# lab-cosmo/torch-pme

Hardware: AMD Instinct MI355X
Metric: atom-steps/sec (energy+forces) (higher is better)
Workload: dtype f32

## Files before the change

torch-pme_amd/csrc/bricks_device.h:

```cpp
#ifndef MIPME_BRICKS_DEVICE_H
#define MIPME_BRICKS_DEVICE_H
#include <algorithm>
#include <cmath>
#include <cstdlib>

#include <rocprim/device/device_radix_sort.hpp>

#include "host.h"
#include <map>
#include <utility>

#include "rows_body.h"
#include "fft_lds.h"

namespace mipme {

static constexpr int BRICK = 8;
static constexpr int BRICK_PTS = BRICK * BRICK * BRICK;

#define MIPME_SGPR_CAP __attribute__((amdgpu_num_sgpr(80)))
static inline int spread_stage_rows(int order, size_t real_bytes);
static inline size_t spread_row_reals(int, size_t) { return 3 * BRICK; }

struct BrickGeom {
  int nbx, nby, nbz, nb;
  int xcd;
};

static inline BrickGeom make_brick_geom(const mipme_mesh_t* m) {
  BrickGeom b;
  b.nbx = (m->nx + BRICK - 1) / BRICK;
  b.nby = (m->ny + BRICK - 1) / BRICK;
  b.nbz = (m->nz + BRICK - 1) / BRICK;
  b.nb = b.nbx * b.nby * b.nbz;
  b.xcd = 1;
  return b;
}
static inline unsigned brick_grid(const BrickGeom& b) { return b.xcd ? pad8(unsigned(b.nb)) : unsigned(b.nb); }
__device__ __forceinline__ unsigned brick_of(const BrickGeom& b, unsigned wg) {
  return b.xcd ? xcd_contiguous(wg, unsigned(b.nb)) : wg;
}

__device__ __forceinline__ int wrap1(int a, int n) {
  a += a < 0 ? n : 0;
  return a >= n ? a - n : a;
}

struct BinsLayout {
  size_t snap, over_brick, rec, wts, codes, qs, plist, pover, wmax, epart, dst, det, det_sort_bytes, total;
  int cap;
  int pcap;
  int64_t slots;
};

static bool deterministic_mode() {
  static const bool on = env_flag("MIPME_DETERMINISTIC", false);
  return on;
}
static constexpr int kRowsPerSpreadBlock = 512 / kRowLanes;
static constexpr int kSpreadWaves = 512 / 64;

static inline int bin_capacity(int nb, int64_t N) {
  const int64_t mean = (N + nb - 1) / nb;
  int64_t cap = (4 * mean + 8 + 7) / 8 * 8;
  const int64_t all = (N + 7) / 8 * 8;
  if (cap > all) cap = all;
  return int(cap < 8 ? 8 : cap);
}

template <int N, typename T>
constexpr int wts_stride() {
  constexpr int V = 16 / int(sizeof(T));
  return (6 * N + V - 1) / V * V;
}
static inline size_t wts_stride_rt(int order, size_t elem) { return (6 * size_t(order) * elem + 15) / 16 * 16 / elem; }

template <int N, typename T>
__device__ __forceinline__ void store_slot_weights(T* __restrict__ wr, const T (&wx)[N], const T (&wy)[N], const T (&wz)[N],
                                                   const T (&dwx)[N], const T (&dwy)[N], const T (&dwz)[N]) {
  constexpr int W = wts_stride<N, T>(), V = 16 / int(sizeof(T));
  struct alignas(16) Chunk {
    T e[V];
  };
  T v[W];
#pragma unroll
  for (int t = 0; t < N; ++t) {
    v[t] = wx[t];
    v[N + t] = wy[t];
    v[2 * N + t] = wz[t];
    v[3 * N + t] = dwx[t];
    v[4 * N + t] = dwy[t];
    v[5 * N + t] = dwz[t];
  }
#pragma unroll
  for (int t = 6 * N; t < W; ++t) v[t] = T(0);
  Chunk* d = reinterpret_cast<Chunk*>(wr);
#pragma unroll
  for (int k = 0; k < W / V; ++k) {
    Chunk c;
#pragma unroll
    for (int e = 0; e < V; ++e) c.e[e] = v[k * V + e];
    d[k] = c;
  }
}

template <int N, typename T>
constexpr int plane_entry_words() {
  constexpr int V = 16 / int(sizeof(T));
  return (3 + N + V - 1) / V * V;
}
static inline size_t plane_entry_bytes_rt(int order, size_t elem) { return ((3 + size_t(order)) * elem + 15) / 16 * 16; }
static constexpr int kPlanePackBits = 10;

static int plane_list_capacity(const mipme_mesh_t* m, int64_t N, int dtype);
static inline BinsLayout bins_layout(const mipme_mesh_t* m, int64_t N, int dtype) {
  const BrickGeom b = make_brick_geom(m);
  const size_t s = dtype == MIPME_F32 ? 4 : 8;
  auto al = [](size_t x) { return (x + 255) & ~size_t(255); };
  BinsLayout l;
  l.cap = bin_capacity(b.nb, N);
  l.slots = int64_t(b.nb) * l.cap + N;
  size_t off = 0;
  l.snap = off;       off += al(sizeof(int) * size_t(b.nb + 1));
  l.over_brick = off; off += al(sizeof(int) * size_t(N));
  l.rec = off;        off += al(sizeof(int4) * size_t(l.slots));
  l.wts = off;        off += al(wts_stride_rt(m->order, s) * s * size_t(l.slots));
  l.codes = off;      off += al(size_t(l.slots));
  l.qs = off;         off += al(s * size_t(l.slots));
  l.pcap = plane_list_capacity(m, N, dtype);
  l.plist = off;      off += al(plane_entry_bytes_rt(m->order, s) * size_t(l.pcap) * size_t(l.pcap ? m->nx * kPlaneSub : 0));
  l.pover = off;      off += al(plane_entry_bytes_rt(m->order, s) * size_t(l.pcap ? N : 0));
  l.wmax = off;       off += al(sizeof(float) * size_t(l.pcap ? (N + 63) / 64 : 0));
  l.epart = off; off += al(2 * sizeof(double) * kSpreadWaves * (((size_t(N) + kRowsPerSpreadBlock - 1) / kRowsPerSpreadBlock + 1) & ~size_t(1)));
  l.dst = off;        off += al(sizeof(int) * size_t(N));
  l.det = off;
  l.det_sort_bytes = 0;
  if (deterministic_mode()) {
    size_t sb = 0;
    unsigned* nul = nullptr;
    (void)rocprim::radix_sort_pairs(nullptr, sb, nul, nul, nul, nul, size_t(N > 0 ? N : 1), 0u, 32u, hipStream_t(0), false);
    l.det_sort_bytes = sb;
    off += 6 * al(sizeof(int) * size_t(N > 0 ? N : 1)) + al(sb);
  }
  l.total = off;
  return l;
}

struct BinIndex {
  int* live;
  int* snap;
  const int* over_brick;
  int nb, cap;
  int64_t over_base;
  unsigned char* codes = nullptr;
  int* plive = nullptr;
  int pband_shift = -1;
  void* plist = nullptr;
  void* pover = nullptr;
  int pcap = 0;
  float* wmax = nullptr;
  int n_wmax = 0;
};

template <int N>
__device__ __forceinline__ unsigned reach_code(const int (&m)[3], int nx, int ny, int nz) {
  constexpr int s0 = stencil_start<N>();
  const int n[3] = {nx, ny, nz};
  unsigned code = 0;
#pragma unroll
  for (int d = 0; d < 3; ++d) {
    const int i = m[d] & (BRICK - 1), size = min(BRICK, n[d] - (m[d] & ~(BRICK - 1)));
    code |= (i + s0 < 0 ? 1u : 0u) << (2 * d);
    code |= (i + s0 + N - 1 >= size ? 2u : 0u) << (2 * d);
  }
  return code;
}

__device__ __forceinline__ void split_runtime(double u, bool even, int& m, double& x) {
  if (even) {
    const double fl = floor(u);
    m = int(fl);
    x = u - (fl + 0.5);
  } else {
    const double r = rint(u);
    m = int(r);
    x = u - r;
  }
}

template <typename T>
__device__ __forceinline__ void atom_mesh_coords(const Geom& g, bool even, const T* __restrict__ pos, int64_t i,
                                                 int (&m)[3], double (&x)[3]) {
  const double rx = double(pos[3 * i + 0]), ry = double(pos[3 * i + 1]), rz = double(pos[3 * i + 2]);
  const double u[3] = {double(g.nx) * (rx * g.inv[0] + ry * g.inv[3] + rz * g.inv[6]),
                       double(g.ny) * (rx * g.inv[1] + ry * g.inv[4] + rz * g.inv[7]),
                       double(g.nz) * (rx * g.inv[2] + ry * g.inv[5] + rz * g.inv[8])};
  const int n[3] = {g.nx, g.ny, g.nz};
#pragma unroll
  for (int d = 0; d < 3; ++d) {
    int mm;
    split_runtime(u[d], even, mm, x[d]);
    m[d] = posmod(mm, n[d]);
  }
}

static constexpr int64_t kCoalescedBinAtoms = 100000;
template <int SCHEME, int N, typename T, bool COALESCE = false, bool LEAN = false>
__device__ __forceinline__ void bin_atoms_body(const Geom& g, const BrickGeom& bg, const BinIndex& bi, int64_t Natoms,
                                               const T* __restrict__ pos, int* __restrict__ over_brick,
                                               int4* __restrict__ rec, T* __restrict__ wts, const T* __restrict__ q,
                                               AtomRecord<T>* __restrict__ atom_rec, unsigned block,
                                               const int* __restrict__ slot_of = nullptr, T* __restrict__ qs = nullptr,
                                               int* __restrict__ slot_dst = nullptr) {
  static_assert(!(LEAN && COALESCE), "the lean binning pass has no weight rows to stage");
  const int64_t i = int64_t(block) * blockDim.x + threadIdx.x;
  const bool valid = i < Natoms;
  const int lane = threadIdx.x & 63;
  int b = -1;
  int m[3] = {0, 0, 0};
  double x[3] = {0.0, 0.0, 0.0};
  if (valid) {
    atom_mesh_coords<T>(g, (N % 2) == 0, pos, i, m, x);
    b = ((m[0] / BRICK) * bg.nby + m[1] / BRICK) * bg.nbz + m[2] / BRICK;
  }
  int myslot = 0, over_k = -1;
  int pl_leader = lane, pl_rank = 0, pl_count = 0, pl_slot = -1;
  const int pl_key = bi.pband_shift >= 0 ? ((m[1] >> bi.pband_shift) & (kPlaneSub - 1))
                                         : int(((int64_t(block) * blockDim.x + threadIdx.x) >> 6) & (kPlaneSub - 1));
  const int pl_list = m[0] * kPlaneSub + pl_key;
  if (slot_of) {
    if (valid) {
      myslot = slot_of[i];
      if (myslot >= bi.cap) over_k = myslot - bi.cap;
    }
  } else {
    unsigned long long remaining = __ballot(valid);
    int my_leader = lane, my_rank = 0, my_count = 0;
    while (remaining) {
      const int leader = __ffsll((long long)remaining) - 1;
      const int b0 = __shfl(b, leader, 64);
      const unsigned long long peers = __ballot(valid && b == b0);
      if (valid && b == b0) {
        my_leader = leader;
        my_rank = __popcll(peers & ((1ull << lane) - 1ull));
        my_count = __popcll(peers);
      }
      remaining &= ~peers;
    }
    if (bi.plive && bi.wmax && qs) {
      float a = valid ? fabsf(float(q[i])) : 0.f;
      a = fmaxf(a, dpp_mov<0xB1>(a));
      a = fmaxf(a, dpp_mov<0x4E>(a));
      a = fmaxf(a, dpp_mov<0x141>(a));
      a = fmaxf(a, dpp_mov<0x140>(a));
      a = fmaxf(fmaxf(read_lane(a, 0), read_lane(a, 16)), fmaxf(read_lane(a, 32), read_lane(a, 48)));
      if (lane == 0) bi.wmax[(int64_t(block) * blockDim.x + threadIdx.x) >> 6] = a;
    }
    if (bi.plive) {
      unsigned long long rem = __ballot(valid);
      while (rem) {
        const int leader = __ffsll((long long)rem) - 1;
        const int p0 = __shfl(pl_list, leader, 64);
        const unsigned long long peers = __ballot(valid && pl_list == p0);
        if (valid && pl_list == p0) {
          pl_leader = leader;
          pl_rank = __popcll(peers & ((1ull << lane) - 1ull));
          pl_count = __popcll(peers);
        }
        rem &= ~peers;
      }
    }
    int base = 0, pbase = 0;
    if (valid && my_leader == lane) base = atomicAdd(&bi.live[b], my_count);
    if (bi.plive && valid && pl_leader == lane) pbase = atomicAdd(&bi.plive[pl_list], pl_count);
    base = __shfl(base, my_leader, 64);
    myslot = base + my_rank;
    if (bi.plive) pl_slot = __shfl(pbase, pl_leader, 64) + pl_rank;
  }
  int64_t dst = 0;
  if (valid) {
    if (myslot < bi.cap) {
      dst = int64_t(b) * bi.cap + myslot;
    } else {
      const int k = over_k >= 0 ? over_k : atomicAdd(&bi.live[bi.nb], 1);
      over_brick[k] = b;
      dst = bi.over_base + k;
    }
    if (atom_rec) {
      AtomRecord<T> r;
      r.x = pos[3 * i];
      r.y = pos[3 * i + 1];
      r.z = pos[3 * i + 2];
      r.w = q[i];
      atom_rec[i] = r;
    }
    if constexpr (LEAN) {
      slot_dst[i] = int(dst);
    } else {
      rec[dst] = make_int4(m[0], m[1], m[2], int(i));
      if (qs) qs[dst] = q[i];
      if (bi.codes && dst < bi.over_base) bi.codes[dst] = (unsigned char)reach_code<N>(m, g.nx, g.ny, g.nz);
    }
  }
  constexpr int W = wts_stride<N, T>();
  auto store_plane_entry = [&](const T (&wx)[N]) __attribute__((always_inline)) {
    if (!valid || pl_slot < 0) return;
    constexpr int EW = plane_entry_words<N, T>(), V = 16 / int(sizeof(T));
    struct alignas(16) Chunk {
      T e[V];
    };
    T* e;
    if (pl_slot < bi.pcap)
      e = (T*)bi.plist + (int64_t(pl_list) * bi.pcap + pl_slot) * EW;
    else
      e = (T*)bi.pover + int64_t(atomicAdd(&bi.plive[g.nx * kPlaneSub], 1)) * EW;
    T v[EW];
    const int packed = (m[0] << (2 * kPlanePackBits)) | (m[1] << kPlanePackBits) | m[2];
    if constexpr (sizeof(T) == 4)
      v[0] = __int_as_float(packed);
    else
      v[0] = __longlong_as_double((long long)packed);
    v[1] = T(x[1]);
    v[2] = T(x[2]);
    const T qa = q[i];
#pragma unroll
    for (int t = 0; t < N; ++t) v[3 + t] = qa * wx[t];
#pragma unroll
    for (int t = 3 + N; t < EW; ++t) v[t] = T(0);
    Chunk* d = reinterpret_cast<Chunk*>(e);
#pragma unroll
    for (int k = 0; k < EW / V; ++k) {
      Chunk c;
#pragma unroll
      for (int u = 0; u < V; ++u) c.e[u] = v[k * V + u];
      d[k] = c;
    }
  };
  constexpr bool STAGED = COALESCE && sizeof(T) * 64 * W * (256 / 64) <= 48 * 1024;
  if constexpr (STAGED) {
    __shared__ T sw[256 / 64][64 * W];
    T* mine = sw[threadIdx.x >> 6] + lane * W;
#pragma unroll
    for (int d = 0; d < 3; ++d) {
      T w[N], dw[N];
      weights_1d<SCHEME, N, true, T>(T(x[d]), w, dw);
#pragma unroll
      for (int t = 0; t < N; ++t) {
        mine[d * N + t] = w[t];
        mine[(3 + d) * N + t] = dw[t];
      }
      if (d == 0 && bi.plive) store_plane_entry(w);
    }
    __builtin_amdgcn_fence(__ATOMIC_RELEASE, "wavefront");
    __builtin_amdgcn_wave_barrier();
    constexpr int PER = 64 / W;
    const unsigned long long vmask = __ballot(valid);
    const int sub = lane / W, k = lane % W;
    const T* rows = sw[threadIdx.x >> 6];
    for (int a0 = 0; a0 < 64; a0 += PER) {
      const int j = a0 + (sub < PER ? sub : 0);
      const int64_t dj = __shfl(dst, j < 64 ? j : 0, 64);
      if (sub < PER && k < 6 * N && j < 64 && ((vmask >> j) & 1ull)) wts[dj * W + k] = rows[j * W + k];
    }
  } else if constexpr (LEAN) {
    if (!valid) return;
    T wx[N], dwx[N];
    weights_1d<SCHEME, N, false, T>(T(x[0]), wx, dwx);
    if (bi.plive) store_plane_entry(wx);
  } else {
    if (!valid) return;
    T wx[N], wy[N], wz[N], dwx[N], dwy[N], dwz[N];
    weights_1d<SCHEME, N, true, T>(T(x[0]), wx, dwx);
    weights_1d<SCHEME, N, true, T>(T(x[1]), wy, dwy);
    weights_1d<SCHEME, N, true, T>(T(x[2]), wz, dwz);
    store_slot_weights<N, T>(wts + dst * W, wx, wy, wz, dwx, dwy, dwz);
    if (bi.plive) store_plane_entry(wx);
  }
}

template <int SCHEME, int N, typename T, bool COALESCE>
__global__ __launch_bounds__(256) void bin_atoms_kernel(Geom g, BrickGeom bg, BinIndex bi, int64_t Natoms,
                                                       const T* __restrict__ pos, int* __restrict__ over_brick,
                                                       int4* __restrict__ rec, T* __restrict__ wts,
                                                       const T* __restrict__ q, AtomRecord<T>* __restrict__ atom_rec,
                                                       const int* __restrict__ slot_of, T* __restrict__ qs) {
  bin_atoms_body<SCHEME, N, T, COALESCE>(g, bg, bi, Natoms, pos, over_brick, rec, wts, q, atom_rec, blockIdx.x, slot_of, qs);
}

template <int SCHEME, int N, typename T>
__global__ __launch_bounds__(256) void bin_atoms_lean_kernel(Geom g, BrickGeom bg, BinIndex bi, int64_t Natoms,
                                                            const T* __restrict__ pos, int* __restrict__ over_brick,
                                                            const T* __restrict__ q, AtomRecord<T>* __restrict__ atom_rec,
                                                            T* __restrict__ qs, int* __restrict__ slot_dst) {
  bin_atoms_body<SCHEME, N, T, false, true>(g, bg, bi, Natoms, pos, over_brick, nullptr, nullptr, q, atom_rec, blockIdx.x, nullptr,
                                            qs, slot_dst);
}

#ifndef MIPME_SLOT_RIDER_ATOMS
#define MIPME_SLOT_RIDER_ATOMS 256
#endif
static constexpr int kSlotRiderAtoms = MIPME_SLOT_RIDER_ATOMS;
template <int SCHEME, int N, typename T>
__device__ __forceinline__ void slot_rider_body(const SlotRider& r, unsigned rider) {
  if (int(threadIdx.x) >= r.per_rider) return;
  const int64_t i = int64_t(rider) * r.per_rider + threadIdx.x;
  if (i >= r.n_atoms) return;
  const T* __restrict__ pos = static_cast<const T*>(r.pos);
  const T* __restrict__ q = static_cast<const T*>(r.q);
  const int64_t dst = r.dst[i];
  int m[3];
  double x[3];
  atom_mesh_coords<T>(r.g, (N % 2) == 0, pos, i, m, x);
  r.rec[dst] = make_int4(m[0], m[1], m[2], int(i));
  static_cast<T*>(r.qs)[dst] = q[i];
  if (dst < r.over_base) r.codes[dst] = (unsigned char)reach_code<N>(m, r.g.nx, r.g.ny, r.g.nz);
  T wx[N], wy[N], wz[N], dwx[N], dwy[N], dwz[N];
  weights_1d<SCHEME, N, true, T>(T(x[0]), wx, dwx);
  weights_1d<SCHEME, N, true, T>(T(x[1]), wy, dwy);
  weights_1d<SCHEME, N, true, T>(T(x[2]), wz, dwz);
  store_slot_weights<N, T>(static_cast<T*>(r.wts) + dst * wts_stride<N, T>(), wx, wy, wz, dwx, dwy, dwz);
}

template <typename T>
__global__ __launch_bounds__(256) void det_keys_kernel(Geom g, BrickGeom bg, bool even, int64_t Natoms, const T* __restrict__ pos,
                                                      unsigned* __restrict__ keys, unsigned* __restrict__ vals) {
  const int64_t i = int64_t(blockIdx.x) * blockDim.x + threadIdx.x;
  if (i >= Natoms) return;
  int m[3];
  double x[3];
  atom_mesh_coords<T>(g, even, pos, i, m, x);
  keys[i] = unsigned(((m[0] / BRICK) * bg.nby + m[1] / BRICK) * bg.nbz + m[2] / BRICK);
  vals[i] = unsigned(i);
}

static __global__ __launch_bounds__(256) void det_slots_kernel(int64_t Natoms, int cap, const unsigned* __restrict__ keys2,
                                                       const unsigned* __restrict__ vals2, int* __restrict__ slot_of,
                                                       int* __restrict__ over_flag, int* __restrict__ live) {
  const int64_t p = int64_t(blockIdx.x) * blockDim.x + threadIdx.x;
  if (p >= Natoms) return;
  const unsigned b = keys2[p];
  int64_t lo = 0, hi = p;
  while (lo < hi) {
    const int64_t mid = (lo + hi) >> 1;
    if (keys2[mid] < b)
      lo = mid + 1;
    else
      hi = mid;
  }
  const int slot = int(p - lo);
  slot_of[vals2[p]] = slot;
  over_flag[p] = slot >= cap ? 1 : 0;
  if (slot == 0) {
    int64_t l2 = p, h2 = Natoms;
    while (l2 < h2) {
      const int64_t mid = (l2 + h2) >> 1;
      if (keys2[mid] <= b)
        l2 = mid + 1;
      else
        h2 = mid;
    }
    live[b] = int(l2 - p);
  }
}

static __global__ __launch_bounds__(1024) void det_overflow_kernel(int64_t Natoms, int cap, int nb, const unsigned* __restrict__ vals2,
                                                           const int* __restrict__ over_flag, int* __restrict__ slot_of,
                                                           int* __restrict__ live) {
  __shared__ int part[1024];
  const int t = threadIdx.x;
  const int64_t per = (Natoms + 1023) / 1024;
  const int64_t lo = min(int64_t(t) * per, Natoms), hi = min(lo + per, Natoms);
  int sum = 0;
  for (int64_t k = lo; k < hi; ++k) sum += over_flag[k];
  part[t] = sum;
  __syncthreads();
  for (int off = 1; off < 1024; off <<= 1) {
    const int v = t >= off ? part[t - off] : 0;
    __syncthreads();
    part[t] += v;
    __syncthreads();
  }
// ... 470 lines not shown
  extern __shared__ __attribute__((aligned(16))) char smem_rows[];
  if (cs.brick) {
    const unsigned b = brick_of(sa.bg, cs.slot);
    if (cs.slot < n_pad && b < n_spread) spread_brick_body<N, T>(sa, b);
  } else if (cs.slot < n_rows_pad) {
    const unsigned r = sa.bg.xcd ? xcd_contiguous(cs.slot, n_row_blocks) : cs.slot;
    if (r < n_row_blocks) cosched_row_block<T, PFAST, COMPACT, CELL>(ra, r, smem_rows);
  }
#ifdef MIPME_WG_TIMELINE
  __syncthreads();
#endif
  MIPME_WG_STAMP(1);
}

template <int N, typename T, int PFAST, bool COMPACT, bool CELL = false>
__global__ __launch_bounds__(SPREAD_THREADS, (sizeof(T) == 4 && COMPACT) ? (CELL ? MIPME_CELL_WAVES : 6) : 1) void spread_rows_kernel(
    SpreadArgs<T> sa, FusedRowsArgs<T> ra, unsigned n_spread, unsigned pattern) {
  spread_rows_body<N, T, PFAST, COMPACT, CELL>(sa, ra, n_spread, pattern);
}
template <int N, typename T, int PFAST, bool COMPACT, bool CELL = false>
__global__ __launch_bounds__(SPREAD_THREADS, (sizeof(T) == 4 && COMPACT) ? (CELL ? MIPME_CELL_WAVES : 6) : 1) MIPME_SGPR_CAP void spread_rows_capped_kernel(
    SpreadArgs<T> sa, FusedRowsArgs<T> ra, unsigned n_spread, unsigned pattern) {
  spread_rows_body<N, T, PFAST, COMPACT, CELL>(sa, ra, n_spread, pattern);
}
template <int N, typename T, bool CELL>
constexpr bool spread_rows_sgpr_capped() {
#ifdef MIPME_SGPR_CAP_OFF
  return false;
#else
  return sizeof(T) == 4 && N == 5 && !CELL;
#endif
}

template <typename T, int PFAST, bool COMPACT, bool CELL = false>
__global__ __launch_bounds__(256) void rows_only_kernel(FusedRowsArgs<T> ra, int xcd) {
  constexpr bool F64_BODY = COMPACT && std::is_same<T, double>::value && (PFAST == 1 || PFAST == 6) && kRowLanes == 16;
  __shared__ __attribute__((aligned(16))) char tab_raw[F64_BODY ? kRowsF64LdsBytes : sizeof(AtomRecord<T>) * kShiftTableSize];
  AtomRecord<T>* tab = reinterpret_cast<AtomRecord<T>*>(tab_raw);
  constexpr int BS = 256;
  const unsigned n_row_blocks = unsigned((ra.N + BS / kRowLanes - 1) / (BS / kRowLanes));
  const unsigned r = xcd ? xcd_contiguous(blockIdx.x, n_row_blocks) : blockIdx.x;
  if (r >= n_row_blocks) return;
  if constexpr (COMPACT && std::is_same<T, float>::value) {
    if (CELL || !ra.dist_out) {
      sr_rows_pk_body<PFAST, BS, CELL>(ra, r, tab);
      return;
    }
  }
#if MIPME_ROW_LANES == 16
  if constexpr (F64_BODY) {
    if (CELL || !ra.dist_out) {
      sr_rows_f64_body<BS, CELL, PFAST>(ra, r, tab_raw);
      return;
    }
  }
#endif
  if constexpr (!CELL) sr_fused_rows_body<T, kPotForce, false, PFAST, false, true, BS, 0, COMPACT>(ra, r, tab);
}

template <typename T>
static inline bool rows_cell_supported(int pfast, int shift_format, const void* dist_out) {
  if ((shift_format & kShiftFormatMask) != kShiftTable32 || dist_out || kRowLanes != 16) return false;
  return pfast == 1 || pfast == 6;
}

template <typename T>
struct PlaneArgs {
  Cplx<T>* hat = nullptr;
  int logny = 0, loglz = 0;
  int tile_off = 0, tw_off = 0;
  int misc_off = 0;
  int parts = 1;
  Cplx<T>* hat_more = nullptr;
  int64_t more_stride = 0;
  int band_rows = 0, bands = 1;
};

static constexpr size_t kPlaneLdsCosched = 39 * 1024;
static inline size_t plane_tile_bytes(int ny, int nz, size_t real_bytes) { return 2 * real_bytes * size_t(ny) * (size_t(nz / 2) + 1); }
static inline size_t plane_tw_bytes(int ny, int nz, size_t real_bytes) {
  const size_t Lz = size_t(nz / 2), Ltab = size_t(ny) > Lz ? size_t(ny) : Lz;
  return 2 * real_bytes * (Ltab / 2 + (Lz + 1));
}
template <typename T>
static inline void plane_lds_layout(int rows, int nz, PlaneArgs<T>& pa, size_t& total, bool ystage = true) {
  const size_t acc = sizeof(double) * size_t(rows) * nz, tile = plane_tile_bytes(rows, nz, sizeof(T));
  const size_t tile_off = sizeof(T) == 4 ? 0 : acc;
  const size_t tw_off = sizeof(T) == 4 ? (acc > tile ? acc : tile) : acc + tile;
  pa.tile_off = int(tile_off);
  pa.tw_off = int(tw_off);
  pa.misc_off = int(tw_off + plane_tw_bytes(ystage ? rows : 0, nz, sizeof(T)));
  total = size_t(pa.misc_off) + 640;
}
static inline int plane_band_rows(const mipme_mesh_t* m, int dtype) {
  static const bool bands_env = env_flag("MIPME_PLANE_BANDS", true);
  for (int rows = m->ny; rows >= 4 && rows * kPlaneSub >= m->ny; rows >>= 1) {
    size_t need = 0;
    if (dtype == MIPME_F32) {
      PlaneArgs<float> pa;
      plane_lds_layout<float>(rows, m->nz, pa, need, rows == m->ny);
    } else {
      PlaneArgs<double> pa;
      plane_lds_layout<double>(rows, m->nz, pa, need, rows == m->ny);
    }
    if (need <= kPlaneLdsCosched) return rows;
    if (!bands_env) break;
  }
  return 0;
}
static inline bool plane_fits_cosched(const mipme_mesh_t* m, int dtype) { return plane_band_rows(m, dtype) == m->ny; }

static inline bool sparse_bricks(int64_t n_atoms, int nb);
static int plane_list_capacity(const mipme_mesh_t* m, int64_t N, int dtype) {
  static const bool plane_env = env_flag("MIPME_PLANE_SPREAD", true);
  if (!plane_env || deterministic_mode() || m->n_channels != 1 || N <= 0) return 0;
  const bool pow2 = (m->ny & (m->ny - 1)) == 0 && (m->nz & (m->nz - 1)) == 0 && m->nz >= 4 && m->ny >= 2;
  if (!pow2 || m->nx < 2 * BRICK) return 0;
  if (m->nx > (1 << 11) || m->ny > (1 << kPlanePackBits) || m->nz > (1 << kPlanePackBits)) return 0;
  if (sparse_bricks(N, make_brick_geom(m).nb)) return 0;
  const int band_rows = plane_band_rows(m, dtype);
  if (band_rows == 0) return 0;
  if (band_rows < m->ny && m->ny / kPlaneSub < 8) return 0;
  const int64_t lists = int64_t(m->nx) * kPlaneSub, mean = (N + lists - 1) / lists, all = (N + 15) / 16 * 16;
  int64_t cap = (4 * mean + 32 + 15) / 16 * 16;
  if (cap > all) cap = all;
  return int(cap);
}

template <int N, typename T>
struct PlaneItem {
  T vx;
  int my, mz;
  T wy[N], wz[N];
};

template <int N, typename T>
struct PlaneRaw {
  T w[plane_entry_words<N, T>()];
};

template <int N, typename T>
__device__ __forceinline__ void plane_raw_load(PlaneRaw<N, T>& r, bool ok, const T* __restrict__ base, int64_t idx) {
  constexpr int EW = plane_entry_words<N, T>(), V = 16 / int(sizeof(T));
  struct alignas(16) Chunk {
    T e[V];
  };
  const Chunk* src = reinterpret_cast<const Chunk*>(base + (ok ? idx : 0) * EW);
#pragma unroll
  for (int k = 0; k < EW / V; ++k) {
    const Chunk c = src[k];
#pragma unroll
    for (int u = 0; u < V; ++u) r.w[k * V + u] = c.e[u];
  }
#pragma unroll
  for (int t = 3; t < EW; ++t) r.w[t] = ok ? r.w[t] : T(0);
}
template <typename T>
__device__ __forceinline__ int plane_raw_packed(T w0) {
  if constexpr (sizeof(T) == 4)
    return __float_as_int(w0);
  else
    return int(__double_as_longlong(w0));
}

template <int SCHEME, int N, typename T>
__device__ __forceinline__ void plane_item_make(PlaneItem<N, T>& it, const PlaneRaw<N, T>& r, int tt, T scale) {
  const int packed = plane_raw_packed(r.w[0]);
  it.my = (packed >> kPlanePackBits) & ((1 << kPlanePackBits) - 1);
  it.mz = packed & ((1 << kPlanePackBits) - 1);
  T qwx[N], unused[N];
#pragma unroll
  for (int t = 0; t < N; ++t) qwx[t] = r.w[3 + t];
  it.vx = pick<N, T>(qwx, tt) * scale;
  weights_1d<SCHEME, N, false, T>(r.w[1], it.wy, unused);
  weights_1d<SCHEME, N, false, T>(r.w[2], it.wz, unused);
}

static constexpr unsigned kFxMagicHi = 0x43380000u;
template <int N, typename T, bool BANDED>
__device__ __forceinline__ void plane_item_scatter(double* __restrict__ acc, const Geom& g, const PlaneItem<N, T>& it, double fx_scale,
                                                   int row_lo, int rows) {
  constexpr int s0 = stencil_start<N>();
  int zo[N];
#pragma unroll
  for (int k = 0; k < N; ++k) zo[k] = wrap1(it.mz + s0 + k, g.nz);
#pragma unroll
  for (int j = 0; j < N; ++j) {
    int r = wrap1(it.my + s0 + j, g.ny);
    if constexpr (BANDED) {
      r -= row_lo;
      if (unsigned(r) >= unsigned(rows)) continue;
    }
    const int row = r * g.nz;
    const T ay = it.vx * it.wy[j];
#pragma unroll
    for (int k = 0; k < N; ++k) {
      if constexpr (sizeof(T) == 4) {
        const double t = __builtin_fma(double(ay * it.wz[k]), fx_scale, 6755399441055744.0);
        const unsigned long long bits = (unsigned long long)__double_as_longlong(t) - ((unsigned long long)kFxMagicHi << 32);
        atomicAdd(reinterpret_cast<unsigned long long*>(&acc[row + zo[k]]), bits);
      } else {
        atomicAdd(&acc[row + zo[k]], double(ay * it.wz[k]));
      }
    }
  }
}

template <int SCHEME, int N, typename T, bool BANDED = false>
__device__ __forceinline__ void plane_spread_yz_body(const SpreadArgs<T>& args, const PlaneArgs<T>& pa, unsigned item,
                                                     char* smem) {
  constexpr bool banded = BANDED;
  const int n_bands = banded ? pa.bands : 1;
  const unsigned unit = item / unsigned(pa.parts);
  const int part = int(item - unit * unsigned(pa.parts));
  const unsigned plane = banded ? unit / unsigned(n_bands) : unit;
  const int band = banded ? int(unit - plane * unsigned(n_bands)) : 0;
  const Geom& g = args.g;
  const int rows = banded ? pa.band_rows : g.ny, row_lo = band * rows;
  const BinIndex& bins = args.bins;
  const T* __restrict__ plist = (const T*)bins.plist;
  const T* __restrict__ pover = (const T*)bins.pover;
  const int tid = threadIdx.x, nthr = blockDim.x;
  constexpr int s0 = stencil_start<N>();
  MIPME_WG_PHASE(0);
  double* acc = reinterpret_cast<double*>(smem);
  const int npts = rows * g.nz;
  const int x0 = int(plane);
  const int spb = kPlaneSub / n_bands;
  const int SUBS = banded ? min(spb + 2, kPlaneSub) : kPlaneSub;
  const int sub0 = banded ? band * spb - 1 : 0;
  const int NL = N * SUBS;
  auto list_of = [&](int l) __attribute__((always_inline)) {
    return posmod(x0 - s0 - l / SUBS, g.nx) * kPlaneSub + ((sub0 + (l % SUBS)) & (kPlaneSub - 1));
  };
  int my_count = 0;
  if (tid < NL) my_count = bins.plive[list_of(tid)];
  float my_wmax = 0.f;
  if (sizeof(T) == 4 && tid < bins.n_wmax) my_wmax = bins.wmax[tid];
  for (int i = tid; i < npts; i += nthr) acc[i] = 0.0;
  const YzTile<T> yt = banded ? yz_tile_setup<T, false>(rows, g.nz, smem + pa.tile_off, smem + pa.tw_off)
                              : yz_tile_setup<T, true>(g.ny, g.nz, smem + pa.tile_off, smem + pa.tw_off);
  if (args.from_live) {
    const int n_items = g.nx * n_bands * pa.parts;
    for (int b = int(item) + tid * n_items; b <= bins.nb; b += n_items * nthr) bins.snap[b] = bin_count_of(bins, b, true);
  }
  int* lst = reinterpret_cast<int*>(smem + pa.misc_off);
  static_assert(N * kPlaneSub < 64, "bookkeeping of the plane lists");
  double* fxs = reinterpret_cast<double*>(lst + 128);
  float* wred = reinterpret_cast<float*>(lst + 132);
  if constexpr (sizeof(T) == 4) {
    float a = my_wmax;
    bool bad = !(my_wmax == my_wmax);
    for (int i = tid + nthr; i < bins.n_wmax; i += nthr) {
      const float w = bins.wmax[i];
      bad |= !(w == w);
      a = fmaxf(a, w);
    }
    a = fmaxf(a, dpp_mov<0xB1>(a));
    a = fmaxf(a, dpp_mov<0x4E>(a));
    a = fmaxf(a, dpp_mov<0x141>(a));
    a = fmaxf(a, dpp_mov<0x140>(a));
    a = fmaxf(fmaxf(read_lane(a, 0), read_lane(a, 16)), fmaxf(read_lane(a, 32), read_lane(a, 48)));
    if (__builtin_amdgcn_ballot_w64(bad) != 0) a = __builtin_nanf("");
    if ((tid & 63) == 0) wred[tid >> 6] = a;
  }
  if (tid < NL) lst[64 + tid] = min(my_count, bins.pcap);
  __syncthreads();
  if (tid <= NL) {
    int run = 0;
    for (int u = 0; u < tid; ++u) run += lst[64 + u];
    lst[tid] = run;
  }
  if constexpr (sizeof(T) == 4) {
    if (tid == 64) {
      float qmax = 0.f;
      bool bad = false;
      for (int w = 0; w < (nthr >> 6); ++w) {
        bad |= !(wred[w] == wred[w]);
        qmax = fmaxf(qmax, wred[w]);
      }
      int n_atoms = bins.plive[g.nx * kPlaneSub] + 1;
      for (int u = 0; u < NL; ++u) n_atoms += lst[64 + u];
      int e = 0;
      const double bd = double(qmax) * 1.00001 * fabs(double(args.scale)) * double(n_atoms);
      (void)frexp(bd, &e);
      const bool finite = !bad && bd == bd && bd < 1e300;
      fxs[0] = finite ? ldexp(1.0, 50 - e) : __builtin_nan("");
      fxs[1] = finite ? ldexp(1.0, e - 50) : __builtin_nan("");
    }
  }
  __syncthreads();
  MIPME_WG_PHASE(1);
  const double fx_scale = sizeof(T) == 4 ? fxs[0] : 1.0;
  auto guard_item = [&](const PlaneItem<N, T>& it) __attribute__((always_inline)) {
    if constexpr (sizeof(T) == 4) {
      const T chk = it.vx * it.wy[0] * it.wz[0];
      if (!(__builtin_fabsf(chk) <= 3.0e38f)) fxs[1] = __builtin_nan("");
    }
  };
  const int total = lst[NL];
  const int lo = int(int64_t(total) * part / pa.parts), hi = int(int64_t(total) * (part + 1) / pa.parts);
  const int n_batches = (hi - lo + nthr - 1) / nthr;
  auto entry_of = [&](int b, int& tt) __attribute__((always_inline)) -> int64_t {
    const int gidx = lo + b * nthr + tid;
    int l = 0;
    for (int u = 1; u < NL; ++u) l += gidx >= lst[u] ? 1 : 0;
    tt = l / SUBS;
    if (b >= n_batches || gidx >= hi) return -1;
    return int64_t(list_of(l)) * bins.pcap + (gidx - lst[l]);
  };
  int tt0 = 0, tt1 = 0;
  PlaneRaw<N, T> r0, r1;
  {
    const int64_t e0 = entry_of(0, tt0), e1 = entry_of(1, tt1);
    plane_raw_load<N, T>(r0, e0 >= 0, plist, e0);
    plane_raw_load<N, T>(r1, e1 >= 0, plist, e1);
  }
  for (int b = 0; b < n_batches; ++b) {
    int tt2 = 0;
    const int64_t e2 = entry_of(b + 2, tt2);
    PlaneRaw<N, T> r2;
    plane_raw_load<N, T>(r2, e2 >= 0, plist, e2);
    PlaneItem<N, T> cur;
    plane_item_make<SCHEME, N, T>(cur, r0, tt0, args.scale);
    if (cur.vx != T(0)) {
      guard_item(cur);
      plane_item_scatter<N, T, BANDED>(acc, g, cur, fx_scale, row_lo, rows);
    }
    r0 = r1;
    tt0 = tt1;
    r1 = r2;
    tt1 = tt2;
  }
  if (part == 0) {
    const int oc = bins.plive[g.nx * kPlaneSub];
    for (int i = tid; i < oc; i += nthr) {
      PlaneRaw<N, T> r;
      plane_raw_load<N, T>(r, true, pover, i);
      int d = x0 - (plane_raw_packed(r.w[0]) >> (2 * kPlanePackBits)) - s0;
      d += d < 0 ? g.nx : 0;
      d -= d >= g.nx ? g.nx : 0;
      if (d < N) {
        PlaneItem<N, T> it;
        plane_item_make<SCHEME, N, T>(it, r, d, args.scale);
        guard_item(it);
        plane_item_scatter<N, T, BANDED>(acc, g, it, fx_scale, row_lo, rows);
      }
    }
  }
  __syncthreads();
  MIPME_WG_PHASE(2);
  const double fx_inv = sizeof(T) == 4 ? fxs[1] : 1.0;
  {
    const int Lz = yt.Lz, RZ = yt.RZ, npairs = rows * Lz;
    constexpr int CH = 4;
    for (int base = 0; base < npairs; base += CH * nthr) {
      Cplx<T> v[CH];
#pragma unroll
      for (int u = 0; u < CH; ++u) {
        const int idx = base + u * nthr + tid;
        if constexpr (sizeof(T) == 4) {
          const long long* ai = reinterpret_cast<const long long*>(acc);
          v[u] = idx < npairs ? Cplx<T>{T(double(ai[2 * idx]) * fx_inv), T(double(ai[2 * idx + 1]) * fx_inv)} : Cplx<T>{T(0), T(0)};
        } else {
          v[u] = idx < npairs ? Cplx<T>{T(acc[2 * idx]), T(acc[2 * idx + 1])} : Cplx<T>{T(0), T(0)};
        }
      }
      __syncthreads();
#pragma unroll
      for (int u = 0; u < CH; ++u) {
        const int idx = base + u * nthr + tid;
        if (idx < npairs) {
          const int y = idx / Lz, j = idx - y * Lz;
          const int jr = pa.loglz ? int(__brev(unsigned(j)) >> (32 - pa.loglz)) : 0;
          yt.tile[y * RZ + jr] = v[u];
        }
      }
      __syncthreads();
    }
  }
  MIPME_WG_PHASE(3);
  Cplx<T>* dst = part == 0 ? pa.hat : pa.hat_more + int64_t(part - 1) * pa.more_stride;
  if (banded)
    yz_forward_finish<T, false>(yt, rows, g.nz, 0, pa.loglz, dst + (int64_t(plane) * g.ny + row_lo) * yt.RZ);
  else
    yz_forward_finish<T, true>(yt, g.ny, g.nz, pa.logny, pa.loglz, dst + int64_t(plane) * g.ny * yt.RZ);
  MIPME_WG_PHASE(4);
}

template <int SCHEME, int N, typename T, bool BANDED = false>
__global__ __launch_bounds__(1024) void plane_spread_kernel(SpreadArgs<T> sa, PlaneArgs<T> pa) {
  MIPME_SKIP_IF_SET(sa.skip);
  extern __shared__ __attribute__((aligned(16))) char smem_plane[];
  plane_spread_yz_body<SCHEME, N, T, BANDED>(sa, pa, blockIdx.x, smem_plane);
}

template <int SCHEME, int N, typename T, int PFAST, bool COMPACT, bool CELL, bool BANDED>
__device__ __forceinline__ void plane_rows_body(const SpreadArgs<T>& sa, const PlaneArgs<T>& pa, const FusedRowsArgs<T>& ra,
                                                unsigned n_planes, unsigned n_row_blocks) {
  MIPME_WG_STAMP(0);
  extern __shared__ __attribute__((aligned(16))) char smem_pr[];
  const unsigned n_pad = pad8(n_planes);
  if (blockIdx.x < n_pad) {
    const unsigned p = xcd_contiguous(blockIdx.x, n_planes);
    if (p < n_planes) plane_spread_yz_body<SCHEME, N, T, BANDED>(sa, pa, p, smem_pr);
  } else {
    const unsigned r = xcd_contiguous(blockIdx.x - n_pad, n_row_blocks);
    if (r < n_row_blocks) cosched_row_block<T, PFAST, COMPACT, CELL>(ra, r, smem_pr);
  }
#ifdef MIPME_WG_TIMELINE
  __syncthreads();
#endif
  MIPME_WG_STAMP(1);
}
template <int SCHEME, int N, typename T, int PFAST, bool COMPACT, bool CELL = false, bool BANDED = false>
__global__ __launch_bounds__(SPREAD_THREADS, (sizeof(T) == 4 && COMPACT) ? (CELL ? MIPME_CELL_WAVES : 6) : 1) void plane_rows_kernel(
    SpreadArgs<T> sa, PlaneArgs<T> pa, FusedRowsArgs<T> ra, unsigned n_planes ,
    unsigned n_row_blocks) {
  plane_rows_body<SCHEME, N, T, PFAST, COMPACT, CELL, BANDED>(sa, pa, ra, n_planes, n_row_blocks);
}
template <int SCHEME, int N, typename T, int PFAST, bool COMPACT, bool CELL = false, bool BANDED = false>
__global__ __launch_bounds__(SPREAD_THREADS, (sizeof(T) == 4 && COMPACT) ? (CELL ? MIPME_CELL_WAVES : 6) : 1) MIPME_SGPR_CAP void plane_rows_capped_kernel(
    SpreadArgs<T> sa, PlaneArgs<T> pa, FusedRowsArgs<T> ra, unsigned n_planes, unsigned n_row_blocks) {
  plane_rows_body<SCHEME, N, T, PFAST, COMPACT, CELL, BANDED>(sa, pa, ra, n_planes, n_row_blocks);
}

static constexpr int GATHER_THREADS = 512;

static constexpr int GATHER_THREADS_SPARSE = 128;
static constexpr int kSparseBrickAtoms = 40;
static constexpr int kSparseMinBricks = 4096;
static inline bool sparse_bricks(int64_t n_atoms, int nb) {
  static const bool force = env_flag("MIPME_SPARSE_FORCE", false);
  return force || (n_atoms <= int64_t(kSparseBrickAtoms) * nb && nb >= kSparseMinBricks);
}

template <int N, int NT, typename T, int THREADS = GATHER_THREADS>
__device__ __forceinline__ void load_tiles(const Geom& g, int ox, int oy, int oz, const T* __restrict__ m0,
                                           const T* __restrict__ m1, T* tile) {
  constexpr int TL = BRICK + N - 1;
  constexpr int s0 = stencil_start<N>();
  const int64_t plane = int64_t(g.ny) * g.nz;
  for (int k = threadIdx.x; k < TL * TL * TL; k += THREADS) {
    const int tx = k / (TL * TL), ty = (k / TL) % TL, tz = k % TL;
    const int gx = wrap1(ox + s0 + tx, g.nx), gy = wrap1(oy + s0 + ty, g.ny), gz = wrap1(oz + s0 + tz, g.nz);
    const int64_t gi = gx * plane + int64_t(gy) * g.nz + gz;
    tile[k] = m0[gi];
    if constexpr (NT == 2) tile[TL * TL * TL + k] = m1[gi];
  }
}

static constexpr int kGatherLanes = 8;

template <typename T>
struct GatherTail {
  const T* force;
  T force_scale;
  const T* seed;
  T* grad_pos;
  T* energy;
  const double* epart_sr;
  const double* epart_k;
  int n_sr, n_k;
  T* grad_q;
  double* rpart;
  const AtomRecord<T>* rec4;
  const T* aux_seed;
  const int* live_flags;
  double* elog = nullptr;
  int* elog_cursor = nullptr;
  int elog_cap = 0, elog_stride = 1;
  const double* slab_mom = nullptr;
  double slab_c0 = 0.0, slab_L = 0.0;
  int slab_axis = 0;
};
template <typename T>
__device__ __forceinline__ T slab_coord(const AtomRecord<T>& r, int axis) {
  return axis == 0 ? r.x : (axis == 1 ? r.y : r.z);
}
template <typename T>
static GatherTail<T> make_gather_tail(const GatherTailHost& th, const double* epart_sr, int n_sr, const void* rec4,
                                      const void* live_flags) {
  GatherTail<T> tail;
  tail.force = (const T*)th.force;
  tail.force_scale = T(th.force_scale);
// ... 464 lines not shown
```

Baseline: 588.5 million.

## Store precomputed y/z weights in fat plane entries and use wave-uniform list lookup

For f32 with order up to 5, plane-list entries now carry the precomputed y and z B-spline weights alongside the charge-scaled x weights, so the plane scatter no longer recomputes weights_1d per item. The list-index lookup in the scatter loop is rewritten with a wavefront ballot and readlane instead of a per-thread linear scan over the shared boundary array. The prefetch depth drops from two to one for fat entries to limit register pressure. In exchange entries are larger, which raises memory traffic and the plane-list footprint.

```diff
diff --git a/torch-pme_amd/csrc/bricks_device.h b/torch-pme_amd/csrc/bricks_device.h
--- a/torch-pme_amd/csrc/bricks_device.h
+++ b/torch-pme_amd/csrc/bricks_device.h
@@ -104,12 +104,29 @@
   }
 }
 
+#ifndef MIPME_PLANE_FAT_F64
+#define MIPME_PLANE_FAT_F64 0
+#endif
+#ifndef MIPME_PLANE_FAT_F32
+#define MIPME_PLANE_FAT_F32 1
+#endif
+static constexpr int kPlaneFatMaxOrder = 5;
+constexpr bool plane_entry_fat_rt(int order, size_t elem) {
+  return order <= kPlaneFatMaxOrder && (elem == 4 ? MIPME_PLANE_FAT_F32 != 0 : MIPME_PLANE_FAT_F64 != 0);
+}
+template <int N, typename T>
+constexpr bool plane_entry_fat() {
+  return plane_entry_fat_rt(N, sizeof(T));
+}
 template <int N, typename T>
 constexpr int plane_entry_words() {
   constexpr int V = 16 / int(sizeof(T));
-  return (3 + N + V - 1) / V * V;
-}
-static inline size_t plane_entry_bytes_rt(int order, size_t elem) { return ((3 + size_t(order)) * elem + 15) / 16 * 16; }
+  return ((plane_entry_fat<N, T>() ? 1 + 3 * N : 3 + N) + V - 1) / V * V;
+}
+static inline size_t plane_entry_bytes_rt(int order, size_t elem) {
+  const size_t words = plane_entry_fat_rt(order, elem) ? 1 + 3 * size_t(order) : 3 + size_t(order);
+  return (words * elem + 15) / 16 * 16;
+}
 static constexpr int kPlanePackBits = 10;
 
 static int plane_list_capacity(const mipme_mesh_t* m, int64_t N, int dtype);
@@ -306,6 +323,7 @@
   auto store_plane_entry = [&](const T (&wx)[N]) __attribute__((always_inline)) {
     if (!valid || pl_slot < 0) return;
     constexpr int EW = plane_entry_words<N, T>(), V = 16 / int(sizeof(T));
+    constexpr bool FAT = plane_entry_fat<N, T>();
     struct alignas(16) Chunk {
       T e[V];
     };
@@ -320,13 +338,27 @@
       v[0] = __int_as_float(packed);
     else
       v[0] = __longlong_as_double((long long)packed);
-    v[1] = T(x[1]);
-    v[2] = T(x[2]);
     const T qa = q[i];
-#pragma unroll
-    for (int t = 0; t < N; ++t) v[3 + t] = qa * wx[t];
-#pragma unroll
-    for (int t = 3 + N; t < EW; ++t) v[t] = T(0);
+    if constexpr (FAT) {
+      T wy[N], wz[N], unused[N];
+      T oy = T(x[1]), oz = T(x[2]);
+      asm volatile("" : "+v"(oy), "+v"(oz));
+      weights_1d<SCHEME, N, false, T>(oy, wy, unused);
+      weights_1d<SCHEME, N, false, T>(oz, wz, unused);
+#pragma unroll
+      for (int t = 0; t < N; ++t) {
+        v[1 + t] = qa * wx[t];
+        v[1 + N + t] = wy[t];
+        v[1 + 2 * N + t] = wz[t];
+      }
+    } else {
+      v[1] = T(x[1]);
+      v[2] = T(x[2]);
+#pragma unroll
+      for (int t = 0; t < N; ++t) v[3 + t] = qa * wx[t];
+    }
+#pragma unroll
+    for (int t = FAT ? 1 + 3 * N : 3 + N; t < EW; ++t) v[t] = T(0);
     Chunk* d = reinterpret_cast<Chunk*>(e);
 #pragma unroll
     for (int k = 0; k < EW / V; ++k) {
@@ -1103,8 +1135,10 @@
 #pragma unroll
     for (int u = 0; u < V; ++u) r.w[k * V + u] = c.e[u];
   }
-#pragma unroll
-  for (int t = 3; t < EW; ++t) r.w[t] = ok ? r.w[t] : T(0);
+  if constexpr (!plane_entry_fat<N, T>()) {
+#pragma unroll
+    for (int t = 3; t < EW; ++t) r.w[t] = ok ? r.w[t] : T(0);
+  }
 }
 template <typename T>
 __device__ __forceinline__ int plane_raw_packed(T w0) {
@@ -1116,15 +1150,25 @@
 
 template <int SCHEME, int N, typename T>
 __device__ __forceinline__ void plane_item_make(PlaneItem<N, T>& it, const PlaneRaw<N, T>& r, int tt, T scale) {
+  constexpr bool FAT = plane_entry_fat<N, T>();
   const int packed = plane_raw_packed(r.w[0]);
   it.my = (packed >> kPlanePackBits) & ((1 << kPlanePackBits) - 1);
   it.mz = packed & ((1 << kPlanePackBits) - 1);
-  T qwx[N], unused[N];
-#pragma unroll
-  for (int t = 0; t < N; ++t) qwx[t] = r.w[3 + t];
+  T qwx[N];
+#pragma unroll
+  for (int t = 0; t < N; ++t) qwx[t] = r.w[(FAT ? 1 : 3) + t];
   it.vx = pick<N, T>(qwx, tt) * scale;
-  weights_1d<SCHEME, N, false, T>(r.w[1], it.wy, unused);
-  weights_1d<SCHEME, N, false, T>(r.w[2], it.wz, unused);
+  if constexpr (FAT) {
+#pragma unroll
+    for (int t = 0; t < N; ++t) {
+      it.wy[t] = r.w[1 + N + t];
+      it.wz[t] = r.w[1 + 2 * N + t];
+    }
+  } else {
+    T unused[N];
+    weights_1d<SCHEME, N, false, T>(r.w[1], it.wy, unused);
+    weights_1d<SCHEME, N, false, T>(r.w[2], it.wz, unused);
+  }
 }
 
 static constexpr unsigned kFxMagicHi = 0x43380000u;
@@ -1252,36 +1296,58 @@
   const int total = lst[NL];
   const int lo = int(int64_t(total) * part / pa.parts), hi = int(int64_t(total) * (part + 1) / pa.parts);
   const int n_batches = (hi - lo + nthr - 1) / nthr;
+  constexpr bool FAT = plane_entry_fat<N, T>();
+  const int lane = tid & 63;
+  const int lst_lane = lane <= NL ? lst[lane] : 0x7fffffff;
   auto entry_of = [&](int b, int& tt) __attribute__((always_inline)) -> int64_t {
     const int gidx = lo + b * nthr + tid;
-    int l = 0;
-    for (int u = 1; u < NL; ++u) l += gidx >= lst[u] ? 1 : 0;
+    const int g0 = __builtin_amdgcn_readfirstlane(gidx);
+    const int l0 = __builtin_popcountll(__builtin_amdgcn_ballot_w64(lane >= 1 && lane < NL && lst_lane <= g0));
+    int l = l0, first = __builtin_amdgcn_readlane(lst_lane, l0);
+    for (int u = l0 + 1; u < NL; ++u) {
+      const int bnd = __builtin_amdgcn_readlane(lst_lane, u);
+      if (bnd > g0 + 63) break;
+      l += gidx >= bnd ? 1 : 0;
+      first = gidx >= bnd ? bnd : first;
+    }
     tt = l / SUBS;
-    if (b >= n_batches || gidx >= hi) return -1;
-    return int64_t(list_of(l)) * bins.pcap + (gidx - lst[l]);
+    if (b >= n_batches || gidx >= hi) {
+      if constexpr (FAT) tt = -1;
+      return -1;
+    }
+    return int64_t(list_of(l)) * bins.pcap + (gidx - first);
   };
+  constexpr int DEPTH = FAT ? 1 : 2;
   int tt0 = 0, tt1 = 0;
   PlaneRaw<N, T> r0, r1;
   {
-    const int64_t e0 = entry_of(0, tt0), e1 = entry_of(1, tt1);
+    const int64_t e0 = entry_of(0, tt0);
     plane_raw_load<N, T>(r0, e0 >= 0, plist, e0);
-    plane_raw_load<N, T>(r1, e1 >= 0, plist, e1);
+    if constexpr (DEPTH == 2) {
+      const int64_t e1 = entry_of(1, tt1);
+      plane_raw_load<N, T>(r1, e1 >= 0, plist, e1);
+    }
   }
   for (int b = 0; b < n_batches; ++b) {
-    int tt2 = 0;
-    const int64_t e2 = entry_of(b + 2, tt2);
-    PlaneRaw<N, T> r2;
-    plane_raw_load<N, T>(r2, e2 >= 0, plist, e2);
+    int ttn = 0;
+    const int64_t en = entry_of(b + DEPTH, ttn);
+    PlaneRaw<N, T> rn;
+    plane_raw_load<N, T>(rn, en >= 0, plist, en);
     PlaneItem<N, T> cur;
     plane_item_make<SCHEME, N, T>(cur, r0, tt0, args.scale);
     if (cur.vx != T(0)) {
       guard_item(cur);
       plane_item_scatter<N, T, BANDED>(acc, g, cur, fx_scale, row_lo, rows);
     }
-    r0 = r1;
-    tt0 = tt1;
-    r1 = r2;
-    tt1 = tt2;
+    if constexpr (DEPTH == 2) {
+      r0 = r1;
+      tt0 = tt1;
+      r1 = rn;
+      tt1 = ttn;
+    } else {
+      r0 = rn;
+      tt0 = ttn;
+    }
   }
   if (part == 0) {
     const int oc = bins.plive[g.nx * kPlaneSub];
```

Result: faster. 599.8 million, median of 6 (+1.9%).
